# llm-d/llm-d-workload-variant-autoscaler

Hardware: AMD Instinct MI355X
Metric: desired-replica accuracy + SLO-attainment %, Llama-3-8B synthetic QPS ramp (higher is better)
Workload: dtype bf16; 1 GPU; model=meta-llama/Llama-3.1-8B, global_batch=256, seq_len=150, parallelism=dp1, device=AMD Radeon Graphics

## Files before the change

### wva_amd/ops/csrc/attention.hip

```cpp
#include "common.h"
#include "launch.h"

#include <type_traits>

#define HEAD_DIM 128
#define MAX_G 8
#define TILE 64
#define NUM_WAVES 4
#define ROW_DW 66
#define S_ROW 65

template <bool KV_FP8>
using kv_elem_t = std::conditional_t<KV_FP8, fp8_t, bf16>;

__device__ __forceinline__ long ws_row_offset(int b, int kvh, int g, int split,
                                              int num_kv_heads, int G,
                                              int num_splits) {
  return ((((long)b * num_kv_heads + kvh) * G + g) * num_splits + split) *
         (2 + HEAD_DIM);
}

__device__ __forceinline__ long pack8_fp8(const float* v, float inv_scale) {
  unsigned int lo = 0, hi = 0;
  lo = __builtin_amdgcn_cvt_pk_fp8_f32(v[0] * inv_scale, v[1] * inv_scale,
                                       lo, false);
  lo = __builtin_amdgcn_cvt_pk_fp8_f32(v[2] * inv_scale, v[3] * inv_scale,
                                       lo, true);
  hi = __builtin_amdgcn_cvt_pk_fp8_f32(v[4] * inv_scale, v[5] * inv_scale,
                                       hi, false);
  hi = __builtin_amdgcn_cvt_pk_fp8_f32(v[6] * inv_scale, v[7] * inv_scale,
                                       hi, true);
  return (long)(((unsigned long)hi << 32) | lo);
}

struct QFrags {
  bf16x8_frag bf[4];
  long fp8[4];
  float scale;
};

template <bool KV_FP8>
__device__ __forceinline__ QFrags load_q_frags(const bf16* __restrict__ q,
                                               int b, int kvh, int G,
                                               int num_q_heads, int lane,
                                               int wave, int g, int k0,
                                               float* qmax_lds) {
  QFrags qf;
  qf.scale = 1.0f;
#pragma unroll
  for (int kk = 0; kk < 4; ++kk) qf.fp8[kk] = 0;
  float qv[4][8];
#pragma unroll
  for (int kk = 0; kk < 4; ++kk)
#pragma unroll
    for (int i = 0; i < 8; ++i) qv[kk][i] = 0.0f;
  if (g < G) {
    const bf16* qrow = q + ((long)b * num_q_heads + kvh * G + g) * HEAD_DIM;
#pragma unroll
    for (int kk = 0; kk < 4; ++kk) {
      const short* src = reinterpret_cast<const short*>(qrow + 32 * kk + k0);
#pragma unroll
      for (int i = 0; i < 8; ++i) {
        qf.bf[kk][i] = src[i];
        const bf16 bv = *reinterpret_cast<const bf16*>(&src[i]);
        qv[kk][i] = bf2f(bv);
      }
    }
  } else {
#pragma unroll
    for (int kk = 0; kk < 4; ++kk)
#pragma unroll
      for (int i = 0; i < 8; ++i) qf.bf[kk][i] = 0;
  }
  if constexpr (KV_FP8) {
    float amax = 0.0f;
#pragma unroll
    for (int kk = 0; kk < 4; ++kk)
#pragma unroll
      for (int i = 0; i < 8; ++i) amax = fmaxf(amax, fabsf(qv[kk][i]));
    amax = wave_reduce_max(amax);
    if (lane == 0) qmax_lds[wave] = amax;
    __syncthreads();
    float m0 = qmax_lds[0];
#pragma unroll
    for (int w2 = 1; w2 < NUM_WAVES; ++w2) m0 = fmaxf(m0, qmax_lds[w2]);
    qf.scale = fmaxf(m0 / 448.0f, 1e-12f);
    const float inv = 1.0f / qf.scale;
#pragma unroll
    for (int kk = 0; kk < 4; ++kk) qf.fp8[kk] = pack8_fp8(qv[kk], inv);
    __syncthreads();
  }
  return qf;
}

struct SoftmaxStep {
  float p;
  float corr;
};

__device__ __forceinline__ SoftmaxStep online_softmax_step(
    const float* __restrict__ s_row, int tn, int lane, float& m, float& s) {
  const bool live = lane < tn;
  const float score = live ? s_row[lane] : -INFINITY;
  const float tile_max = wave_reduce_max(score);
  const float m_new = fmaxf(m, tile_max);
  const float p = live ? __expf(score - m_new) : 0.0f;
  const float tile_sum = wave_reduce_sum(p);
  const float corr = (m == -INFINITY) ? 0.0f : __expf(m - m_new);
  s = s * corr + tile_sum;
  m = m_new;
  return {p, corr};
}


struct TilePages {
  int id[4];

  __device__ __forceinline__ int pick(int group) const {
    return group == 0 ? id[0] : group == 1 ? id[1] : group == 2 ? id[2] : id[3];
  }
};

__device__ __forceinline__ TilePages load_tile_pages(
    const int* __restrict__ table_row, int t0, int ctx, int block_shift,
    int num_blocks) {
  const int last_block = (ctx - 1) >> block_shift;
  TilePages pages;
#pragma unroll
  for (int g = 0; g < 4; ++g) {
    const int entry = min((t0 + 16 * g) >> block_shift, last_block);
    const int id = table_row[entry];
    pages.id[g] = min(max(id, 0), num_blocks - 1);
  }
  return pages;
}

template <typename T>
__device__ __forceinline__ const T* page_row(const T* head0,
                                             const TilePages& pages, int group,
                                             int pos, int block_mask,
                                             long page_stride) {
  return head0 + (long)pages.pick(group) * page_stride +
         (long)(pos & block_mask) * HEAD_DIM;
}

template <bool KV_FP8, bool PAGED>
__global__ __launch_bounds__(256, 2) void gqa_decode_attn_v4_kernel(
    bf16* __restrict__ out,
    float* __restrict__ workspace,
    const bf16* __restrict__ q,
    const void* __restrict__ k_cache,
    const void* __restrict__ v_cache,
    const int* __restrict__ context_lens,
    const int num_q_heads,
    const int num_kv_heads,
    const int max_seq,
    const float scale,
    const int* __restrict__ block_tables,
    const int max_blocks,
    const int block_shift,
    const int num_blocks) {
  const int b = blockIdx.x;
  const int kvh = blockIdx.y;
  const int split = blockIdx.z;
  const int num_splits = gridDim.z;
  const int G = num_q_heads / num_kv_heads;
  const int ctx =
      PAGED ? min(context_lens[b], max_seq) : context_lens[b];

  const int lane = threadIdx.x & (WAVE_SIZE - 1);
  const int wave = threadIdx.x / WAVE_SIZE;
  const int frag_col = lane % 16;
  const int frag_k0 = 8 * (lane / 16);

  __shared__ float s_smem[MAX_G][S_ROW];
  __shared__ unsigned int v_smem[TILE * ROW_DW];
  __shared__ float p_smem[MAX_G][TILE];
  float* qmax_lds = nullptr;
  if constexpr (KV_FP8) {
    __shared__ float qmax_smem[NUM_WAVES];
    qmax_lds = qmax_smem;
  }

  const QFrags qf = load_q_frags<KV_FP8>(q, b, kvh, G, num_q_heads, lane,
                                         wave, frag_col, frag_k0, qmax_lds);

  const int heads_mine = (G > wave) ? (G - wave + NUM_WAVES - 1) / NUM_WAVES : 0;
  float m[2], s[2], acc[2][2];
#pragma unroll
  for (int j = 0; j < 2; ++j) {
    m[j] = -INFINITY;
    s[j] = 0.0f;
    acc[j][0] = acc[j][1] = 0.0f;
  }

  const long slab_off =
      PAGED ? (long)kvh << (block_shift + 7)
            : ((long)b * num_kv_heads + kvh) * max_seq * HEAD_DIM;
  const long page_stride = (long)num_kv_heads << (block_shift + 7);
  const int block_mask = (1 << block_shift) - 1;
  const int* table_row = block_tables + (long)b * max_blocks;
  const auto* k_slab =
      reinterpret_cast<const kv_elem_t<KV_FP8>*>(k_cache) + slab_off;
  const auto* v_slab =
      reinterpret_cast<const kv_elem_t<KV_FP8>*>(v_cache) + slab_off;

  for (int t0 = split * TILE; t0 < ctx; t0 += num_splits * TILE) {
    const int tn = min(TILE, ctx - t0);
    TilePages pages;
    if constexpr (PAGED)
      pages = load_tile_pages(table_row, t0, ctx, block_shift, num_blocks);

    if constexpr (KV_FP8) {
      const int tile_g8 = tn * (HEAD_DIM / 8);
      const fp8_t* v_src = v_slab + (long)t0 * HEAD_DIM;
      for (int idx = wave * WAVE_SIZE + lane; idx < tile_g8;
           idx += NUM_WAVES * WAVE_SIZE) {
        const int row = idx >> 4;
        const int d8 = (idx & 15) * 8;
        const fp8_t* v_row;
        if constexpr (PAGED)
          v_row = page_row(v_slab, pages,
                           __builtin_amdgcn_readfirstlane(row >> 4), t0 + row,
                           block_mask, page_stride);
        else
          v_row = v_src + (long)row * HEAD_DIM;
        const unsigned short* src =
            reinterpret_cast<const unsigned short*>(v_row + d8);
        unsigned int* dst = &v_smem[row * ROW_DW + d8 / 2];
#pragma unroll
        for (int j = 0; j < 4; ++j) {
          const float2_vt f = unpk2_fp8(src[j]);
          const bf16x2 packed{f2bf(f[0]), f2bf(f[1])};
          dst[j] = *reinterpret_cast<const unsigned int*>(&packed);
        }
      }
    } else {
      typedef __attribute__((ext_vector_type(2))) unsigned int uint2_t;
      const int tile_u2 = tn * (HEAD_DIM / 4);
      const unsigned int* v_src =
          reinterpret_cast<const unsigned int*>(v_slab + (long)t0 * HEAD_DIM);
      for (int idx = wave * WAVE_SIZE + lane; idx < tile_u2;
           idx += NUM_WAVES * WAVE_SIZE) {
        const int row = idx >> 5;
        const int d2 = (idx & 31) * 2;
        const unsigned int* src;
        if constexpr (PAGED)
          src = reinterpret_cast<const unsigned int*>(page_row(
                    v_slab, pages, __builtin_amdgcn_readfirstlane(row >> 4),
                    t0 + row, block_mask, page_stride)) + d2;
        else
          src = &v_src[idx * 2];
        const uint2_t val = *reinterpret_cast<const uint2_t*>(src);
        *reinterpret_cast<uint2_t*>(&v_smem[row * ROW_DW + d2]) = val;
      }
    }

    {
      const int prow = 16 * wave + (lane % 16);
      const int pos = t0 + prow;
      const int pos_lim = PAGED ? ctx : max_seq;
      const int pos_c = pos < pos_lim ? pos : pos_lim - 1;
      const kv_elem_t<KV_FP8>* k_row;
      if constexpr (PAGED)
        k_row = page_row(k_slab, pages, __builtin_amdgcn_readfirstlane(wave),
                         pos_c, block_mask, page_stride);
      else
        k_row = k_slab + (long)pos_c * HEAD_DIM;
      const int k0 = frag_k0;
      f32x4_frag sf = {0.f, 0.f, 0.f, 0.f};
      if constexpr (KV_FP8) {
        const long* ksrc = reinterpret_cast<const long*>(k_row);
        const int l0 = k0 / 8;
#pragma unroll
        for (int kk = 0; kk < 4; ++kk) {
          const long a8 = ksrc[kk * 4 + l0];
          sf = __builtin_amdgcn_mfma_f32_16x16x32_fp8_fp8(
              a8, qf.fp8[kk], sf, 0, 0, 0);
        }
      } else {
#pragma unroll
        for (int kk = 0; kk < 4; ++kk) {
          bf16x8_frag a_frag;
          const short* src =
              reinterpret_cast<const short*>(k_row) + 32 * kk + k0;
#pragma unroll
          for (int i = 0; i < 8; ++i) a_frag[i] = src[i];
          sf = __builtin_amdgcn_mfma_f32_16x16x32_bf16(a_frag, qf.bf[kk],
                                                       sf, 0, 0, 0);
        }
      }
      const float s_eff = KV_FP8 ? scale * qf.scale : scale;
      const int g = lane & 15;
      if (g < G) {
#pragma unroll
        for (int i = 0; i < 4; ++i) {
          const int t = 16 * wave + (lane >> 4) * 4 + i;
          s_smem[g][t] = (t < tn) ? sf[i] * s_eff : -INFINITY;
        }
      }
    }
    __syncthreads();

    for (int j = 0; j < heads_mine; ++j) {
      const int g = wave + j * NUM_WAVES;
      const SoftmaxStep st = online_softmax_step(s_smem[g], tn, lane, m[j], s[j]);
      acc[j][0] *= st.corr;
      acc[j][1] *= st.corr;
      p_smem[g][lane] = st.p;
    }

    for (int j = 0; j < heads_mine; ++j) {
      const int g = wave + j * NUM_WAVES;
      const float* pg = p_smem[g];
      float a0 = acc[j][0], a1 = acc[j][1];
      for (int t = 0; t < tn; ++t) {
        const unsigned int vw = v_smem[t * ROW_DW + lane];
        const bf16x2 vv = *reinterpret_cast<const bf16x2*>(&vw);
        const float p = pg[t];
        a0 = fmaf(p, bf2f(vv.x), a0);
        a1 = fmaf(p, bf2f(vv.y), a1);
      }
      acc[j][0] = a0;
      acc[j][1] = a1;
    }
    __syncthreads();
  }

  if (num_splits == 1) {
    for (int j = 0; j < heads_mine; ++j) {
      const int g = wave + j * NUM_WAVES;
      const float inv = s[j] > 0.0f ? 1.0f / s[j] : 0.0f;
      bf16x2* orow = reinterpret_cast<bf16x2*>(
          out + ((long)b * num_q_heads + kvh * G + g) * HEAD_DIM);
      orow[lane] = bf16x2{f2bf(acc[j][0] * inv), f2bf(acc[j][1] * inv)};
    }
  } else {
    for (int j = 0; j < heads_mine; ++j) {
      const int g = wave + j * NUM_WAVES;
      float* wsp = workspace +
          ws_row_offset(b, kvh, g, split, num_kv_heads, G, num_splits);
      if (lane == 0) {
        wsp[0] = m[j];
        wsp[1] = s[j];
      }
      wsp[2 + 2 * lane] = acc[j][0];
      wsp[2 + 2 * lane + 1] = acc[j][1];
    }
  }
}

template <bool KV_FP8, bool PAGED>
__global__ __launch_bounds__(256, 2) void gqa_decode_attn_v5_kernel(
    bf16* __restrict__ out,
    float* __restrict__ workspace,
    const bf16* __restrict__ q,
    const void* __restrict__ k_cache,
    const void* __restrict__ v_cache,
    const int* __restrict__ context_lens,
    const int num_q_heads,
    const int num_kv_heads,
    const int max_seq,
    const float scale,
    const int* __restrict__ block_tables,
    const int max_blocks,
    const int block_shift,
    const int num_blocks) {
  const int b = blockIdx.x;
  const int kvh = blockIdx.y;
  const int split = blockIdx.z;
  const int num_splits = gridDim.z;
  const int G = num_q_heads / num_kv_heads;
  const int ctx =
      PAGED ? min(context_lens[b], max_seq) : context_lens[b];

  const int lane = threadIdx.x & (WAVE_SIZE - 1);
  const int wave = threadIdx.x / WAVE_SIZE;
  const int frag_col = lane % 16;
  const int frag_k0 = 8 * (lane / 16);

  __shared__ float s_smem[MAX_G][S_ROW];
  __shared__ unsigned int v_smem[TILE * ROW_DW];
  __shared__ float p_smem[MAX_G][TILE];
  __shared__ float corr_smem[MAX_G];
  __shared__ float sum_smem[MAX_G];
  __shared__ float m_smem[MAX_G];
  float* qmax_lds = nullptr;
  if constexpr (KV_FP8) {
    __shared__ float qmax_smem[NUM_WAVES];
    qmax_lds = qmax_smem;
  }

  const QFrags qf = load_q_frags<KV_FP8>(q, b, kvh, G, num_q_heads, lane,
                                         wave, frag_col, frag_k0, qmax_lds);

  const int heads_mine = (G > wave) ? (G - wave + NUM_WAVES - 1) / NUM_WAVES : 0;
  float m[2], s[2];
#pragma unroll
  for (int j = 0; j < 2; ++j) {
    m[j] = -INFINITY;
    s[j] = 0.0f;
  }
  f32x4_frag acc_pv[2] = {f32x4_frag{0.f, 0.f, 0.f, 0.f},
                          f32x4_frag{0.f, 0.f, 0.f, 0.f}};

  const long slab_off =
      PAGED ? (long)kvh << (block_shift + 7)
            : ((long)b * num_kv_heads + kvh) * max_seq * HEAD_DIM;
  const long page_stride = (long)num_kv_heads << (block_shift + 7);
  const int block_mask = (1 << block_shift) - 1;
  const int* table_row = block_tables + (long)b * max_blocks;
  const auto* k_slab =
      reinterpret_cast<const kv_elem_t<KV_FP8>*>(k_cache) + slab_off;
  const auto* v_slab =
      reinterpret_cast<const kv_elem_t<KV_FP8>*>(v_cache) + slab_off;

  for (int t0 = split * TILE; t0 < ctx; t0 += num_splits * TILE) {
    const int tn = min(TILE, ctx - t0);
    TilePages pages;
    if constexpr (PAGED)
      pages = load_tile_pages(table_row, t0, ctx, block_shift, num_blocks);

    if constexpr (KV_FP8) {
      const int tile_g8 = tn * (HEAD_DIM / 8);
      const fp8_t* v_src = v_slab + (long)t0 * HEAD_DIM;
      for (int idx = wave * WAVE_SIZE + lane; idx < tile_g8;
           idx += NUM_WAVES * WAVE_SIZE) {
        const int row = idx >> 4;
        const int d8 = (idx & 15) * 8;
        const fp8_t* v_row;
        if constexpr (PAGED)
          v_row = page_row(v_slab, pages,
                           __builtin_amdgcn_readfirstlane(row >> 4), t0 + row,
                           block_mask, page_stride);
        else
          v_row = v_src + (long)row * HEAD_DIM;
        const unsigned short* src =
            reinterpret_cast<const unsigned short*>(v_row + d8);
        unsigned int* dst = &v_smem[row * ROW_DW + d8 / 2];
#pragma unroll
        for (int j = 0; j < 4; ++j) {
          const float2_vt f = unpk2_fp8(src[j]);
          const bf16x2 packed{f2bf(f[0]), f2bf(f[1])};
          dst[j] = *reinterpret_cast<const unsigned int*>(&packed);
        }
      }
    } else {
      typedef __attribute__((ext_vector_type(2))) unsigned int uint2_t;
      const int tile_u2 = tn * (HEAD_DIM / 4);
      const unsigned int* v_src =
          reinterpret_cast<const unsigned int*>(v_slab + (long)t0 * HEAD_DIM);
      for (int idx = wave * WAVE_SIZE + lane; idx < tile_u2;
           idx += NUM_WAVES * WAVE_SIZE) {
        const int row = idx >> 5;
        const int d2 = (idx & 31) * 2;
        const unsigned int* src;
        if constexpr (PAGED)
          src = reinterpret_cast<const unsigned int*>(page_row(
                    v_slab, pages, __builtin_amdgcn_readfirstlane(row >> 4),
                    t0 + row, block_mask, page_stride)) + d2;
        else
          src = &v_src[idx * 2];
        const uint2_t val = *reinterpret_cast<const uint2_t*>(src);
        *reinterpret_cast<uint2_t*>(&v_smem[row * ROW_DW + d2]) = val;
      }
    }

    {
      const int prow = 16 * wave + (lane % 16);
      const int pos = t0 + prow;
      const int pos_lim = PAGED ? ctx : max_seq;
      const int pos_c = pos < pos_lim ? pos : pos_lim - 1;
      const kv_elem_t<KV_FP8>* k_row;
      if constexpr (PAGED)
        k_row = page_row(k_slab, pages, __builtin_amdgcn_readfirstlane(wave),
                         pos_c, block_mask, page_stride);
      else
        k_row = k_slab + (long)pos_c * HEAD_DIM;
      const int k0 = frag_k0;
      f32x4_frag sf = {0.f, 0.f, 0.f, 0.f};
      if constexpr (KV_FP8) {
        const long* ksrc = reinterpret_cast<const long*>(k_row);
        const int l0 = k0 / 8;
#pragma unroll
        for (int kk = 0; kk < 4; ++kk) {
          const long a8 = ksrc[kk * 4 + l0];
          sf = __builtin_amdgcn_mfma_f32_16x16x32_fp8_fp8(
              a8, qf.fp8[kk], sf, 0, 0, 0);
        }
      } else {
#pragma unroll
        for (int kk = 0; kk < 4; ++kk) {
          bf16x8_frag a_frag;
          const short* src =
              reinterpret_cast<const short*>(k_row) + 32 * kk + k0;
#pragma unroll
          for (int i = 0; i < 8; ++i) a_frag[i] = src[i];
          sf = __builtin_amdgcn_mfma_f32_16x16x32_bf16(a_frag, qf.bf[kk],
                                                       sf, 0, 0, 0);
        }
      }
      const float s_eff = KV_FP8 ? scale * qf.scale : scale;
      const int g = lane & 15;
      if (g < G) {
#pragma unroll
        for (int i = 0; i < 4; ++i) {
          const int t = 16 * wave + (lane >> 4) * 4 + i;
          s_smem[g][t] = (t < tn) ? sf[i] * s_eff : -INFINITY;
        }
      }
    }
    __syncthreads();

    for (int j = 0; j < heads_mine; ++j) {
      const int g = wave + j * NUM_WAVES;
      const SoftmaxStep st = online_softmax_step(s_smem[g], tn, lane, m[j], s[j]);
      p_smem[g][lane] = st.p;
      if (lane == 0) corr_smem[g] = st.corr;
    }
    __syncthreads();

    {
      bf16x8_frag p_frag[2];
#pragma unroll
      for (int kk = 0; kk < 2; ++kk) {
        const int g = lane % 16;
        const int pos0 = 32 * kk + 8 * (lane / 16);
        if (g < G) {
#pragma unroll
          for (int i = 0; i < 8; ++i)
            p_frag[kk][i] = f2bf_bits(p_smem[g][pos0 + i]);
        } else {
#pragma unroll
          for (int i = 0; i < 8; ++i) p_frag[kk][i] = 0;
        }
      }
      const unsigned short* v_u16 =
          reinterpret_cast<const unsigned short*>(v_smem);
#pragma unroll
      for (int nsub = 0; nsub < 2; ++nsub) {
        const int dim = 16 * (wave + 4 * nsub) + (lane % 16);
        f32x4_frag d = acc_pv[nsub];
#pragma unroll
        for (int i = 0; i < 4; ++i) {
          const int h = (lane >> 4) * 4 + i;
          d[i] *= (h < G) ? corr_smem[h] : 0.0f;
        }
#pragma unroll
        for (int kk = 0; kk < 2; ++kk) {
          bf16x8_frag v_frag;
          const int pos0 = 32 * kk + 8 * (lane / 16);
#pragma unroll
          for (int i = 0; i < 8; ++i) {
            const int t = pos0 + i;
            v_frag[i] = (t < tn)
                ? (short)v_u16[(t * ROW_DW + (dim >> 1)) * 2 + (dim & 1)]
                : (short)0;
          }
          d = __builtin_amdgcn_mfma_f32_16x16x32_bf16(p_frag[kk], v_frag, d,
                                                      0, 0, 0);
        }
        acc_pv[nsub] = d;
      }
    }
    __syncthreads();
  }

  for (int j = 0; j < heads_mine; ++j) {
    const int g = wave + j * NUM_WAVES;
    if (lane == 0) {
      sum_smem[g] = s[j];
      m_smem[g] = m[j];
    }
  }
  __syncthreads();

  if (num_splits == 1) {
#pragma unroll
    for (int nsub = 0; nsub < 2; ++nsub) {
      const int dim = 16 * (wave + 4 * nsub) + (lane & 15);
#pragma unroll
      for (int i = 0; i < 4; ++i) {
        const int h = (lane >> 4) * 4 + i;
        if (h >= G) continue;
        const float sv = sum_smem[h];
        const float inv = sv > 0.0f ? 1.0f / sv : 0.0f;
        out[((long)b * num_q_heads + kvh * G + h) * HEAD_DIM + dim] =
            f2bf(acc_pv[nsub][i] * inv);
      }
    }
  } else {
#pragma unroll
    for (int nsub = 0; nsub < 2; ++nsub) {
      const int dim = 16 * (wave + 4 * nsub) + (lane & 15);
#pragma unroll
      for (int i = 0; i < 4; ++i) {
        const int h = (lane >> 4) * 4 + i;
        if (h >= G) continue;
        float* wsp = workspace +
            ws_row_offset(b, kvh, h, split, num_kv_heads, G, num_splits);
        if (wave == 0 && nsub == 0 && (lane & 15) == 0) {
          wsp[0] = m_smem[h];
          wsp[1] = sum_smem[h];
        }
        wsp[2 + dim] = acc_pv[nsub][i];
      }
    }
  }
}

#define MERGE_WAVES 8
__global__ __launch_bounds__(64 * MERGE_WAVES) void gqa_decode_attn_merge_kernel(
    bf16* __restrict__ out,
    const float* __restrict__ workspace,
    const int num_q_heads,
    const int num_kv_heads,
    const int num_splits) {
  const int b = blockIdx.x;
  const int h = blockIdx.y;
  const int G = num_q_heads / num_kv_heads;
  const int kvh = h / G;
  const int g = h % G;
  const int lane = threadIdx.x & 63;
  const int wave = threadIdx.x >> 6;

  __shared__ float sm_m[MERGE_WAVES];
  __shared__ float sm_s[MERGE_WAVES];
  __shared__ float sm_o[MERGE_WAVES][HEAD_DIM];

  const float* base = workspace +
      ws_row_offset(b, kvh, g, 0, num_kv_heads, G, num_splits);
  float M = -INFINITY;
  for (int sp = wave; sp < num_splits; sp += MERGE_WAVES) {
    M = fmaxf(M, base[sp * (2 + HEAD_DIM)]);
  }
  float S = 0.0f, o0 = 0.0f, o1 = 0.0f;
  for (int sp = wave; sp < num_splits; sp += MERGE_WAVES) {
    const float* wsp = base + sp * (2 + HEAD_DIM);
    const float mw = wsp[0];
    if (mw == -INFINITY) continue;
    const float f = __expf(mw - M);
    S += wsp[1] * f;
    o0 = fmaf(wsp[2 + 2 * lane], f, o0);
    o1 = fmaf(wsp[2 + 2 * lane + 1], f, o1);
  }
  if (lane == 0) {
    sm_m[wave] = M;
    sm_s[wave] = S;
  }
  sm_o[wave][2 * lane] = o0;
  sm_o[wave][2 * lane + 1] = o1;
  __syncthreads();

  if (wave != 0) return;
  float Mg = -INFINITY;
  for (int w = 0; w < MERGE_WAVES; ++w) Mg = fmaxf(Mg, sm_m[w]);
  float Sg = 0.0f;
  float g0 = 0.0f, g1 = 0.0f;
  for (int w = 0; w < MERGE_WAVES; ++w) {
    if (sm_m[w] == -INFINITY) continue;
    const float f = __expf(sm_m[w] - Mg);
    Sg += sm_s[w] * f;
    g0 = fmaf(sm_o[w][2 * lane], f, g0);
    g1 = fmaf(sm_o[w][2 * lane + 1], f, g1);
  }
  const float inv = Sg > 0.0f ? 1.0f / Sg : 0.0f;
  bf16x2* orow = reinterpret_cast<bf16x2*>(
      out + ((long)b * num_q_heads + h) * HEAD_DIM);
  orow[lane] = bf16x2{f2bf(g0 * inv), f2bf(g1 * inv)};
}

extern "C" int gqa_decode_attn_num_splits(int batch, int num_kv_heads,
                                          int max_ctx_hint) {
  const int base = batch * num_kv_heads;
  if (base >= 1792) return 1;
  int splits = 1792 / base;
  static int min_tiles = [] {
    const char* e = getenv("WVA_ATTN_MIN_TILES");
    int v = e ? atoi(e) : 8;
    return v > 0 ? v : 8;
  }();
  int cap = 16;
  if (max_ctx_hint > 0) {
    const int by_work = max_ctx_hint / (min_tiles * TILE);
    if (by_work > cap) cap = by_work;
  }
  if (splits > cap) splits = cap;
  const int max_useful = max_ctx_hint > 0 ? (max_ctx_hint + 2 * TILE - 1) / (2 * TILE) : splits;
  if (splits > max_useful && max_useful >= 1) splits = max_useful;
  return splits < 1 ? 1 : splits;
}

template <bool PAGED>
static auto decode_attn_kernel(int variant, int kv_fp8) {
  return variant == 5 ? (kv_fp8 ? gqa_decode_attn_v5_kernel<true, PAGED>
                                : gqa_decode_attn_v5_kernel<false, PAGED>)
                      : (kv_fp8 ? gqa_decode_attn_v4_kernel<true, PAGED>
                                : gqa_decode_attn_v4_kernel<false, PAGED>);
}

extern "C" void launch_gqa_decode_attn(
    void* out, void* workspace, const void* q, const void* k_cache,
    const void* v_cache, const int* context_lens, const PagedKV* paged,
    int batch, int num_q_heads, int num_kv_heads, int max_seq, int num_splits,
    float scale, int variant, int kv_fp8, hipStream_t stream) {
  const auto kernel = !paged ? decode_attn_kernel<false>(variant, kv_fp8)
                             : decode_attn_kernel<true>(variant, kv_fp8);
  const PagedKV p = paged ? *paged : PagedKV{nullptr, 0, 0, 0};
  if (paged) max_seq = p.max_blocks << p.block_shift;
  hipLaunchKernelGGL(kernel, dim3(batch, num_kv_heads, num_splits), dim3(256),
                     0, stream, (bf16*)out, (float*)workspace, (const bf16*)q,
                     k_cache, v_cache, context_lens, num_q_heads, num_kv_heads,
                     max_seq, scale, p.block_tables, p.max_blocks,
                     p.block_shift, p.num_blocks);
  if (num_splits > 1) {
    hipLaunchKernelGGL(gqa_decode_attn_merge_kernel,
                       dim3(batch, num_q_heads), dim3(64 * MERGE_WAVES), 0,
                       stream, (bf16*)out, (const float*)workspace,
                       num_q_heads, num_kv_heads, num_splits);
  }
}
```

### wva_amd/ops/csrc/rmsnorm.hip

```cpp

#include "common.h"
#include "launch.h"

typedef __attribute__((ext_vector_type(4))) float floatx4;

template <bool HAS_RESIDUAL>
__global__ void rmsnorm_kernel(
    bf16* __restrict__ out,
    bf16* __restrict__ residual_out,
    const bf16* __restrict__ input,
    const bf16* __restrict__ residual,
    const bf16* __restrict__ weight,
    const float eps,
    const int hidden) {
  const int row = blockIdx.x;
  const bf16* in_row = input + (long)row * hidden;
  const bf16* res_row = HAS_RESIDUAL ? residual + (long)row * hidden : nullptr;
  bf16* out_row = out + (long)row * hidden;
  bf16* res_out_row =
      HAS_RESIDUAL ? residual_out + (long)row * hidden : nullptr;

  __shared__ float lds_red[16];

  float ss = 0.0f;
  const int vec_n = hidden / 8;
  const bf16x2* in2 = reinterpret_cast<const bf16x2*>(in_row);
  const bf16x2* res2 =
      HAS_RESIDUAL ? reinterpret_cast<const bf16x2*>(res_row) : nullptr;
  bf16x2* res_out2 =
      HAS_RESIDUAL ? reinterpret_cast<bf16x2*>(res_out_row) : nullptr;

  for (int i = threadIdx.x; i < vec_n; i += blockDim.x) {
#pragma unroll
    for (int j = 0; j < 4; ++j) {
      bf16x2 v = in2[i * 4 + j];
      float lo = bf2f(v.x), hi = bf2f(v.y);
      if (HAS_RESIDUAL) {
        bf16x2 r = res2[i * 4 + j];
        lo += bf2f(r.x);
        hi += bf2f(r.y);
        res_out2[i * 4 + j] = bf16x2{f2bf(lo), f2bf(hi)};
      }
      ss = fmaf(lo, lo, ss);
      ss = fmaf(hi, hi, ss);
    }
  }
  ss = block_reduce_sum(ss, lds_red);
  const float inv_rms = rsqrtf(ss / (float)hidden + eps);
  __syncthreads();

  const bf16x2* x2 = HAS_RESIDUAL ? reinterpret_cast<const bf16x2*>(res_out_row)
                                  : in2;
  const bf16x2* w2 = reinterpret_cast<const bf16x2*>(weight);
  bf16x2* o2 = reinterpret_cast<bf16x2*>(out_row);
  for (int i = threadIdx.x; i < vec_n; i += blockDim.x) {
#pragma unroll
    for (int j = 0; j < 4; ++j) {
      bf16x2 v = x2[i * 4 + j];
      bf16x2 w = w2[i * 4 + j];
      o2[i * 4 + j] = bf16x2{
          f2bf(bf2f(v.x) * inv_rms * bf2f(w.x)),
          f2bf(bf2f(v.y) * inv_rms * bf2f(w.y))};
    }
  }
}

extern "C" void launch_rmsnorm(
    void* out, void* residual_out, const void* input, const void* residual,
    const void* weight, float eps, int rows, int hidden, hipStream_t stream) {
  dim3 grid(rows);
  dim3 block(256);
  if (residual != nullptr) {
    hipLaunchKernelGGL(rmsnorm_kernel<true>, grid, block, 0, stream,
                       (bf16*)out, (bf16*)residual_out, (const bf16*)input,
                       (const bf16*)residual, (const bf16*)weight, eps, hidden);
  } else {
    hipLaunchKernelGGL(rmsnorm_kernel<false>, grid, block, 0, stream,
                       (bf16*)out, nullptr, (const bf16*)input, nullptr,
                       (const bf16*)weight, eps, hidden);
  }
}
```

### wva_amd/ops/csrc/rope.hip

```cpp

#include "common.h"
#include "launch.h"

__device__ __forceinline__ void rotate_pair(
    const bf16* src, bf16* dst, int d, int half, int head_dim, float pos,
    float theta) {
  const float inv_freq = __powf(theta, -2.0f * (float)d / (float)head_dim);
  const float angle = pos * inv_freq;
  float c, s;
  __sincosf(angle, &s, &c);
  const float x1 = bf2f(src[d]);
  const float x2 = bf2f(src[d + half]);
  dst[d] = f2bf(x1 * c - x2 * s);
  dst[d + half] = f2bf(x2 * c + x1 * s);
}

struct RopeCosSin {
  float c;
  float s;
};

__device__ __forceinline__ RopeCosSin rope_cos_sin(int d, int head_dim,
                                                   int pos,
                                                   double log2_theta) {
  const double inv_freq =
      exp2(-2.0 * (double)d / (double)head_dim * log2_theta);
  double turns = (double)pos * inv_freq * 0.15915494309189535;
  turns -= floor(turns);
  const float t = (float)turns;
  return {__builtin_amdgcn_cosf(t), __builtin_amdgcn_sinf(t)};
}

struct RopeCosSinCache {
  int d = -1;
  RopeCosSin cs = {1.0f, 0.0f};

  __device__ __forceinline__ RopeCosSin get(int d_new, int head_dim, int pos,
                                            double log2_theta) {
    if (d_new != d) {
      cs = rope_cos_sin(d_new, head_dim, pos, log2_theta);
      d = d_new;
    }
    return cs;
  }
};

__device__ __forceinline__ void rotate_pair_cs(
    const bf16* src, bf16* dst, int d, int half, RopeCosSin cs) {
  const float x1 = bf2f(src[d]);
  const float x2 = bf2f(src[d + half]);
  dst[d] = f2bf(x1 * cs.c - x2 * cs.s);
  dst[d + half] = f2bf(x2 * cs.c + x1 * cs.s);
}

__device__ __forceinline__ long paged_row_offset(
    const int* __restrict__ block_tables, int b, int pos, int max_blocks,
    int block_shift, int num_blocks, int num_kv_heads, int head_dim) {
  const int entry = pos >> block_shift;
  if (pos < 0 || entry >= max_blocks) return -1;
  const int id = block_tables[(long)b * max_blocks + entry];
  if (id < 0 || id >= num_blocks) return -1;
  const long row = (((long)id * num_kv_heads) << block_shift) +
                   (pos & ((1 << block_shift) - 1));
  return row * head_dim;
}

__global__ void rope_kernel(
    bf16* __restrict__ q,
    bf16* __restrict__ k,
    const int* __restrict__ positions,
    const int num_q_heads,
    const int num_k_heads,
    const int head_dim,
    const float theta) {
  const int token = blockIdx.x;
  const float pos = (float)positions[token];
  const int half = head_dim / 2;
  const int total = (num_q_heads + num_k_heads) * half;

  for (int idx = threadIdx.x; idx < total; idx += blockDim.x) {
    const int head = idx / half;
    const int d = idx % half;
    const bool is_q = head < num_q_heads;
    bf16* base = is_q
        ? q + (long)token * num_q_heads * head_dim + (long)head * head_dim
        : k + (long)token * num_k_heads * head_dim +
              (long)(head - num_q_heads) * head_dim;
    rotate_pair(base, base, d, half, head_dim, pos, theta);
  }
}

template <bool PAGED>
__global__ void rope_append_kv_kernel(
    const bf16* __restrict__ qkv,
    bf16* __restrict__ q_out,
    bf16* __restrict__ k_cache,
    bf16* __restrict__ v_cache,
    const int* __restrict__ positions,
    const int num_q_heads,
    const int num_kv_heads,
    const int head_dim,
    const int max_seq,
    const float theta,
    const int* __restrict__ block_tables,
    const int max_blocks,
    const int block_shift,
    const int num_blocks) {
  const int b = blockIdx.x;
  const int pos_i = positions[b];
  const float pos = (float)pos_i;
  const int half = head_dim / 2;
  const long qkv_row = (long)b * (num_q_heads + 2 * num_kv_heads) * head_dim;
  const long row0 =
      PAGED ? paged_row_offset(block_tables, b, pos_i, max_blocks, block_shift,
                               num_blocks, num_kv_heads, head_dim)
            : ((long)b * num_kv_heads * max_seq + pos_i) * head_dim;
  const long head_stride =
      PAGED ? (long)head_dim << block_shift : (long)max_seq * head_dim;
  const bool has_row = !PAGED || row0 >= 0;

  const int rot_total = (num_q_heads + num_kv_heads) * half;
  for (int idx = threadIdx.x; idx < rot_total; idx += blockDim.x) {
    const int head = idx / half;
    const int d = idx % half;
    if (head < num_q_heads) {
      const bf16* src = qkv + qkv_row + (long)head * head_dim;
      bf16* dst = q_out + ((long)b * num_q_heads + head) * head_dim;
      rotate_pair(src, dst, d, half, head_dim, pos, theta);
    } else {
      const int kh = head - num_q_heads;
      const bf16* src = qkv + qkv_row + ((long)num_q_heads + kh) * head_dim;
      bf16* dst = k_cache + row0 + kh * head_stride;
      if (has_row) rotate_pair(src, dst, d, half, head_dim, pos, theta);
    }
  }
  const int v_total = num_kv_heads * half;
  const bf16x2* vsrc = reinterpret_cast<const bf16x2*>(
      qkv + qkv_row + (long)(num_q_heads + num_kv_heads) * head_dim);
  for (int idx = threadIdx.x; idx < v_total; idx += blockDim.x) {
    const int kh = idx / half;
    const int d2 = idx % half;
    bf16x2* dst =
        reinterpret_cast<bf16x2*>(v_cache + row0 + kh * head_stride);
    if (has_row) dst[d2] = vsrc[(long)kh * half + d2];
  }
}

template <bool PAGED>
__global__ void rope_append_kv_fp8_kernel(
    const bf16* __restrict__ qkv,
    bf16* __restrict__ q_out,
    fp8_t* __restrict__ k_cache,
    fp8_t* __restrict__ v_cache,
    const int* __restrict__ positions,
    const int num_q_heads,
    const int num_kv_heads,
    const int head_dim,
    const int max_seq,
    const double log2_theta,
    const int* __restrict__ block_tables,
    const int max_blocks,
    const int block_shift,
    const int num_blocks) {
  const int b = blockIdx.x;
  const int pos_i = positions[b];
  const int half = head_dim / 2;
  const long qkv_row = (long)b * (num_q_heads + 2 * num_kv_heads) * head_dim;
  const long row0 =
      PAGED ? paged_row_offset(block_tables, b, pos_i, max_blocks, block_shift,
                               num_blocks, num_kv_heads, head_dim)
            : ((long)b * num_kv_heads * max_seq + pos_i) * head_dim;
  const long head_stride =
      PAGED ? (long)head_dim << block_shift : (long)max_seq * head_dim;
  const bool has_row = !PAGED || row0 >= 0;

  const int rot_total = (num_q_heads + num_kv_heads) * half;
  RopeCosSinCache cache;
  for (int idx = threadIdx.x; idx < rot_total; idx += blockDim.x) {
    const int head = idx / half;
    const int d = idx % half;
    const RopeCosSin cs = cache.get(d, head_dim, pos_i, log2_theta);
    if (head < num_q_heads) {
      const bf16* src = qkv + qkv_row + (long)head * head_dim;
      bf16* dst = q_out + ((long)b * num_q_heads + head) * head_dim;
      rotate_pair_cs(src, dst, d, half, cs);
    } else {
      const int kh = head - num_q_heads;
      const bf16* src = qkv + qkv_row + ((long)num_q_heads + kh) * head_dim;
      const float x1 = bf2f(src[d]);
      const float x2 = bf2f(src[d + half]);
      fp8_t* dst = k_cache + row0 + kh * head_stride;
      if (has_row) {
        dst[d] = f2fp8(x1 * cs.c - x2 * cs.s);
        dst[d + half] = f2fp8(x2 * cs.c + x1 * cs.s);
      }
    }
  }
  const int v_total = num_kv_heads * half;
  const bf16x2* vsrc = reinterpret_cast<const bf16x2*>(
      qkv + qkv_row + (long)(num_q_heads + num_kv_heads) * head_dim);
  for (int idx = threadIdx.x; idx < v_total; idx += blockDim.x) {
    const int kh = idx / half;
    const int d2 = idx % half;
    const bf16x2 v2 = vsrc[(long)kh * half + d2];
    unsigned short* dst =
        reinterpret_cast<unsigned short*>(v_cache + row0 + kh * head_stride);
    if (has_row) dst[d2] = pk2_fp8(bf2f(v2.x), bf2f(v2.y));
  }
}

extern "C" void launch_rope(
    void* q, void* k, const int* positions, int tokens, int num_q_heads,
    int num_k_heads, int head_dim, float theta, hipStream_t stream) {
  dim3 grid(tokens);
  dim3 block(256);
  hipLaunchKernelGGL(rope_kernel, grid, block, 0, stream, (bf16*)q, (bf16*)k,
                     positions, num_q_heads, num_k_heads, head_dim, theta);
}

template <bool PAGED>
static void launch_append_kernel(
    const void* qkv, void* q_out, void* k_cache, void* v_cache,
    const int* positions, const PagedKV& p, int batch, int num_q_heads,
    int num_kv_heads, int head_dim, int max_seq, float theta, int kv_fp8,
    hipStream_t stream) {
  dim3 grid(batch);
  dim3 block(256);
  if (kv_fp8) {
    hipLaunchKernelGGL(rope_append_kv_fp8_kernel<PAGED>, grid, block, 0,
                       stream, (const bf16*)qkv, (bf16*)q_out, (fp8_t*)k_cache,
                       (fp8_t*)v_cache, positions, num_q_heads, num_kv_heads,
                       head_dim, max_seq, log2((double)theta), p.block_tables,
                       p.max_blocks, p.block_shift, p.num_blocks);
  } else {
    hipLaunchKernelGGL(rope_append_kv_kernel<PAGED>, grid, block, 0, stream,
                       (const bf16*)qkv, (bf16*)q_out, (bf16*)k_cache,
                       (bf16*)v_cache, positions, num_q_heads, num_kv_heads,
                       head_dim, max_seq, theta, p.block_tables, p.max_blocks,
                       p.block_shift, p.num_blocks);
  }
}

extern "C" void launch_rope_append_kv(
    const void* qkv, void* q_out, void* k_cache, void* v_cache,
    const int* positions, const PagedKV* paged, int batch, int num_q_heads,
    int num_kv_heads, int head_dim, int max_seq, float theta, int kv_fp8,
    hipStream_t stream) {
  if (!paged) {
    launch_append_kernel<false>(qkv, q_out, k_cache, v_cache, positions,
                                PagedKV{nullptr, 0, 0, 0}, batch, num_q_heads,
                                num_kv_heads, head_dim, max_seq, theta, kv_fp8,
                                stream);
  } else {
    launch_append_kernel<true>(qkv, q_out, k_cache, v_cache, positions,
                               *paged, batch, num_q_heads, num_kv_heads,
                               head_dim, 0, theta, kv_fp8, stream);
  }
}
```

### wva_amd/ops/csrc/silu_mul.hip

```cpp

#include "common.h"
#include "launch.h"

__global__ void silu_mul_kernel(
    bf16* __restrict__ out,
    const bf16* __restrict__ gate,
    const bf16* __restrict__ up,
    const long n2) {
  const bf16x2* g2 = reinterpret_cast<const bf16x2*>(gate);
  const bf16x2* u2 = reinterpret_cast<const bf16x2*>(up);
  bf16x2* o2 = reinterpret_cast<bf16x2*>(out);
  const long stride = (long)gridDim.x * blockDim.x;
  for (long i = (long)blockIdx.x * blockDim.x + threadIdx.x; i < n2;
       i += stride) {
    bf16x2 g = g2[i];
    bf16x2 u = u2[i];
    const float glo = bf2f(g.x), ghi = bf2f(g.y);
    const float slo = glo / (1.0f + __expf(-glo));
    const float shi = ghi / (1.0f + __expf(-ghi));
    o2[i] = bf16x2{f2bf(slo * bf2f(u.x)), f2bf(shi * bf2f(u.y))};
  }
}

__global__ void silu_mul_fused_kernel(
    bf16* __restrict__ out,
    const bf16* __restrict__ gate_up,
    const long rows,
    const long inter2) {
  const long n2 = rows * inter2;
  const long stride = (long)gridDim.x * blockDim.x;
  bf16x2* o2 = reinterpret_cast<bf16x2*>(out);
  const bf16x2* gu2 = reinterpret_cast<const bf16x2*>(gate_up);
  for (long i = (long)blockIdx.x * blockDim.x + threadIdx.x; i < n2;
       i += stride) {
    const long row = i / inter2;
    const long col = i % inter2;
    const bf16x2 g = gu2[row * 2 * inter2 + col];
    const bf16x2 u = gu2[row * 2 * inter2 + inter2 + col];
    const float glo = bf2f(g.x), ghi = bf2f(g.y);
    const float slo = glo / (1.0f + __expf(-glo));
    const float shi = ghi / (1.0f + __expf(-ghi));
    o2[i] = bf16x2{f2bf(slo * bf2f(u.x)), f2bf(shi * bf2f(u.y))};
  }
}

static int silu_grid(long n2) {
  long want = (n2 + 255) / 256;
  return (int)(want > 8192 ? 8192 : (want < 1 ? 1 : want));
}

extern "C" void launch_silu_mul(
    void* out, const void* gate, const void* up, long n, hipStream_t stream) {
  const long n2 = n / 2;
  hipLaunchKernelGGL(silu_mul_kernel, dim3(silu_grid(n2)), dim3(256), 0,
                     stream, (bf16*)out, (const bf16*)gate, (const bf16*)up,
                     n2);
}

extern "C" void launch_silu_mul_fused(
    void* out, const void* gate_up, long rows, long inter, hipStream_t stream) {
  const long inter2 = inter / 2;
  hipLaunchKernelGGL(silu_mul_fused_kernel, dim3(silu_grid(rows * inter2)),
                     dim3(256), 0, stream, (bf16*)out, (const bf16*)gate_up,
                     rows, inter2);
}
```

Measured before the change: 91.98 %.

## Vectorize rmsnorm, rope, silu_mul kernels and add small-split attention merge

Adds 16-byte vectorized variants of rmsnorm (holding the row in registers so it is read once), rope-append-KV (a shared-memory cos/sin table with 128-bit loads and stores), and silu_mul (plain and fused). It also caches cos/sin per dimension in the scalar rope paths and adds a lighter attention merge kernel that packs four rows per block when the split count is small. Each path is chosen only when pointers are 16-byte aligned and the shapes fit. The aim is fewer memory transactions and less launch and compute overhead in these small, memory-bound kernels. The changes also add more code paths and rely on alignment checks, and the new merge kernel replaces the original merge path whenever the split count is small.

```diff
diff --git a/wva_amd/ops/csrc/attention.hip b/wva_amd/ops/csrc/attention.hip
--- a/wva_amd/ops/csrc/attention.hip
+++ b/wva_amd/ops/csrc/attention.hip
@@ -670,6 +670,36 @@
   orow[lane] = bf16x2{f2bf(g0 * inv), f2bf(g1 * inv)};
 }
 
+#define MERGE_ROWS 4
+__global__ __launch_bounds__(64 * MERGE_ROWS) void gqa_decode_attn_merge_small_kernel(
+    bf16* __restrict__ out,
+    const float* __restrict__ workspace,
+    const int rows,
+    const int num_splits) {
+  const int lane = threadIdx.x & 63;
+  const int row = blockIdx.x * MERGE_ROWS + (threadIdx.x >> 6);
+  if (row >= rows) return;
+  const float* base = workspace + (long)row * num_splits * (2 + HEAD_DIM);
+  float Mg = -INFINITY;
+  for (int sp = 0; sp < num_splits; ++sp) {
+    Mg = fmaxf(Mg, fmaxf(-INFINITY, base[sp * (2 + HEAD_DIM)]));
+  }
+  float Sg = 0.0f;
+  float g0 = 0.0f, g1 = 0.0f;
+  for (int sp = 0; sp < num_splits; ++sp) {
+    const float* wsp = base + sp * (2 + HEAD_DIM);
+    const float m = fmaxf(-INFINITY, wsp[0]);
+    if (m == -INFINITY) continue;
+    const float f = __expf(m - Mg);
+    Sg += wsp[1] * f;
+    g0 = fmaf(wsp[2 + 2 * lane], f, g0);
+    g1 = fmaf(wsp[2 + 2 * lane + 1], f, g1);
+  }
+  const float inv = Sg > 0.0f ? 1.0f / Sg : 0.0f;
+  bf16x2* orow = reinterpret_cast<bf16x2*>(out + (long)row * HEAD_DIM);
+  orow[lane] = bf16x2{f2bf(g0 * inv), f2bf(g1 * inv)};
+}
+
 extern "C" int gqa_decode_attn_num_splits(int batch, int num_kv_heads,
                                           int max_ctx_hint) {
   const int base = batch * num_kv_heads;
@@ -713,7 +743,13 @@
                      k_cache, v_cache, context_lens, num_q_heads, num_kv_heads,
                      max_seq, scale, p.block_tables, p.max_blocks,
                      p.block_shift, p.num_blocks);
-  if (num_splits > 1) {
+  if (num_splits > 1 && num_splits <= MERGE_WAVES) {
+    const int rows = batch * num_q_heads;
+    hipLaunchKernelGGL(gqa_decode_attn_merge_small_kernel,
+                       dim3((rows + MERGE_ROWS - 1) / MERGE_ROWS),
+                       dim3(64 * MERGE_ROWS), 0, stream, (bf16*)out,
+                       (const float*)workspace, rows, num_splits);
+  } else if (num_splits > 1) {
     hipLaunchKernelGGL(gqa_decode_attn_merge_kernel,
                        dim3(batch, num_q_heads), dim3(64 * MERGE_WAVES), 0,
                        stream, (bf16*)out, (const float*)workspace,
diff --git a/wva_amd/ops/csrc/rmsnorm.hip b/wva_amd/ops/csrc/rmsnorm.hip
--- a/wva_amd/ops/csrc/rmsnorm.hip
+++ b/wva_amd/ops/csrc/rmsnorm.hip
@@ -1,3 +1,5 @@
+
+#include <cstdint>
 
 #include "common.h"
 #include "launch.h"
@@ -65,11 +67,114 @@
   }
 }
 
+typedef __attribute__((ext_vector_type(4))) unsigned int u32x4;
+#define RMS_REG_VECS 4
+#define RMS_REG_MAX (RMS_REG_VECS * 256 * 8)
+
+__device__ __forceinline__ float rms_lo(unsigned int w) {
+  return __uint_as_float(w << 16);
+}
+__device__ __forceinline__ float rms_hi(unsigned int w) {
+  return __uint_as_float(w & 0xffff0000u);
+}
+__device__ __forceinline__ unsigned int rms_pack(float lo, float hi) {
+  return (unsigned int)(unsigned short)f2bf_bits(lo) |
+         ((unsigned int)(unsigned short)f2bf_bits(hi) << 16);
+}
+
+template <bool HAS_RESIDUAL>
+__global__ __launch_bounds__(256) void rmsnorm_reg_kernel(
+    bf16* __restrict__ out,
+    bf16* __restrict__ residual_out,
+    const bf16* __restrict__ input,
+    const bf16* __restrict__ residual,
+    const bf16* __restrict__ weight,
+    const float eps,
+    const int hidden) {
+  const int row = blockIdx.x;
+  const int vec_n = hidden / 8;
+  const u32x4* in8 =
+      reinterpret_cast<const u32x4*>(input + (long)row * hidden);
+  const u32x4* res8 = HAS_RESIDUAL ? reinterpret_cast<const u32x4*>(
+                                         residual + (long)row * hidden)
+                                   : nullptr;
+  u32x4* res_out8 = HAS_RESIDUAL ? reinterpret_cast<u32x4*>(
+                                       residual_out + (long)row * hidden)
+                                 : nullptr;
+  const u32x4* w8 = reinterpret_cast<const u32x4*>(weight);
+  u32x4* o8 = reinterpret_cast<u32x4*>(out + (long)row * hidden);
+
+  __shared__ float lds_red[16];
+
+  u32x4 x[RMS_REG_VECS], r[RMS_REG_VECS], w[RMS_REG_VECS];
+#pragma unroll
+  for (int k = 0; k < RMS_REG_VECS; ++k) {
+    const int i = threadIdx.x + 256 * k;
+    if (i < vec_n) {
+      x[k] = in8[i];
+      if (HAS_RESIDUAL) r[k] = res8[i];
+      w[k] = w8[i];
+    }
+  }
+
+  float ss = 0.0f;
+#pragma unroll
+  for (int k = 0; k < RMS_REG_VECS; ++k) {
+    const int i = threadIdx.x + 256 * k;
+    if (i < vec_n) {
+#pragma unroll
+      for (int j = 0; j < 4; ++j) {
+        float lo = rms_lo(x[k][j]), hi = rms_hi(x[k][j]);
+        if (HAS_RESIDUAL) {
+          lo += rms_lo(r[k][j]);
+          hi += rms_hi(r[k][j]);
+          x[k][j] = rms_pack(lo, hi);
+        }
+        ss = fmaf(lo, lo, ss);
+        ss = fmaf(hi, hi, ss);
+      }
+      if (HAS_RESIDUAL) res_out8[i] = x[k];
+    }
+  }
+  ss = block_reduce_sum(ss, lds_red);
+  const float inv_rms = rsqrtf(ss / (float)hidden + eps);
+
+#pragma unroll
+  for (int k = 0; k < RMS_REG_VECS; ++k) {
+    const int i = threadIdx.x + 256 * k;
+    if (i < vec_n) {
+      u32x4 o;
+#pragma unroll
+      for (int j = 0; j < 4; ++j) {
+        o[j] = rms_pack(rms_lo(x[k][j]) * inv_rms * rms_lo(w[k][j]),
+                        rms_hi(x[k][j]) * inv_rms * rms_hi(w[k][j]));
+      }
+      o8[i] = o;
+    }
+  }
+}
+
 extern "C" void launch_rmsnorm(
     void* out, void* residual_out, const void* input, const void* residual,
     const void* weight, float eps, int rows, int hidden, hipStream_t stream) {
   dim3 grid(rows);
   dim3 block(256);
+  const bool aligned =
+      (((uintptr_t)out | (uintptr_t)residual_out | (uintptr_t)input |
+        (uintptr_t)residual | (uintptr_t)weight) & 15) == 0;
+  if (hidden <= RMS_REG_MAX && aligned) {
+    if (residual != nullptr) {
+      hipLaunchKernelGGL(rmsnorm_reg_kernel<true>, grid, block, 0, stream,
+                         (bf16*)out, (bf16*)residual_out, (const bf16*)input,
+                         (const bf16*)residual, (const bf16*)weight, eps,
+                         hidden);
+    } else {
+      hipLaunchKernelGGL(rmsnorm_reg_kernel<false>, grid, block, 0, stream,
+                         (bf16*)out, nullptr, (const bf16*)input, nullptr,
+                         (const bf16*)weight, eps, hidden);
+    }
+    return;
+  }
   if (residual != nullptr) {
     hipLaunchKernelGGL(rmsnorm_kernel<true>, grid, block, 0, stream,
                        (bf16*)out, (bf16*)residual_out, (const bf16*)input,
diff --git a/wva_amd/ops/csrc/rope.hip b/wva_amd/ops/csrc/rope.hip
--- a/wva_amd/ops/csrc/rope.hip
+++ b/wva_amd/ops/csrc/rope.hip
@@ -1,24 +1,52 @@
+
+#include <cstdint>
 
 #include "common.h"
 #include "launch.h"
 
-__device__ __forceinline__ void rotate_pair(
-    const bf16* src, bf16* dst, int d, int half, int head_dim, float pos,
-    float theta) {
+struct RopeCosSin {
+  float c;
+  float s;
+};
+
+__device__ __forceinline__ RopeCosSin rope_cos_sin_f32(int d, int head_dim,
+                                                       float pos,
+                                                       float theta) {
   const float inv_freq = __powf(theta, -2.0f * (float)d / (float)head_dim);
   const float angle = pos * inv_freq;
   float c, s;
   __sincosf(angle, &s, &c);
+  return {c, s};
+}
+
+__device__ __forceinline__ float rope_lo(float x1, float x2, RopeCosSin cs) {
+  return fmaf(cs.c, x1, -__fmul_rn(cs.s, x2));
+}
+__device__ __forceinline__ float rope_hi(float x1, float x2, RopeCosSin cs) {
+  return fmaf(cs.s, x1, __fmul_rn(cs.c, x2));
+}
+
+struct RopeCosSinCacheF32 {
+  int d = -1;
+  RopeCosSin cs = {1.0f, 0.0f};
+
+  __device__ __forceinline__ RopeCosSin get(int d_new, int head_dim,
+                                            float pos, float theta) {
+    if (d_new != d) {
+      cs = rope_cos_sin_f32(d_new, head_dim, pos, theta);
+      d = d_new;
+    }
+    return cs;
+  }
+};
+
+__device__ __forceinline__ void rotate_pair(
+    const bf16* src, bf16* dst, int d, int half, RopeCosSin cs) {
   const float x1 = bf2f(src[d]);
   const float x2 = bf2f(src[d + half]);
-  dst[d] = f2bf(x1 * c - x2 * s);
-  dst[d + half] = f2bf(x2 * c + x1 * s);
-}
-
-struct RopeCosSin {
-  float c;
-  float s;
-};
+  dst[d] = f2bf(rope_lo(x1, x2, cs));
+  dst[d + half] = f2bf(rope_hi(x1, x2, cs));
+}
 
 __device__ __forceinline__ RopeCosSin rope_cos_sin(int d, int head_dim,
                                                    int pos,
@@ -78,6 +106,7 @@
   const int half = head_dim / 2;
   const int total = (num_q_heads + num_k_heads) * half;
 
+  RopeCosSinCacheF32 cache;
   for (int idx = threadIdx.x; idx < total; idx += blockDim.x) {
     const int head = idx / half;
     const int d = idx % half;
@@ -86,7 +115,7 @@
         ? q + (long)token * num_q_heads * head_dim + (long)head * head_dim
         : k + (long)token * num_k_heads * head_dim +
               (long)(head - num_q_heads) * head_dim;
-    rotate_pair(base, base, d, half, head_dim, pos, theta);
+    rotate_pair(base, base, d, half, cache.get(d, head_dim, pos, theta));
   }
 }
 
@@ -120,18 +149,20 @@
   const bool has_row = !PAGED || row0 >= 0;
 
   const int rot_total = (num_q_heads + num_kv_heads) * half;
+  RopeCosSinCacheF32 cache;
   for (int idx = threadIdx.x; idx < rot_total; idx += blockDim.x) {
     const int head = idx / half;
     const int d = idx % half;
+    const RopeCosSin cs = cache.get(d, head_dim, pos, theta);
     if (head < num_q_heads) {
       const bf16* src = qkv + qkv_row + (long)head * head_dim;
       bf16* dst = q_out + ((long)b * num_q_heads + head) * head_dim;
-      rotate_pair(src, dst, d, half, head_dim, pos, theta);
+      rotate_pair(src, dst, d, half, cs);
     } else {
       const int kh = head - num_q_heads;
       const bf16* src = qkv + qkv_row + ((long)num_q_heads + kh) * head_dim;
       bf16* dst = k_cache + row0 + kh * head_stride;
-      if (has_row) rotate_pair(src, dst, d, half, head_dim, pos, theta);
+      if (has_row) rotate_pair(src, dst, d, half, cs);
     }
   }
   const int v_total = num_kv_heads * half;
@@ -143,6 +174,106 @@
     bf16x2* dst =
         reinterpret_cast<bf16x2*>(v_cache + row0 + kh * head_stride);
     if (has_row) dst[d2] = vsrc[(long)kh * half + d2];
+  }
+}
+
+typedef __attribute__((ext_vector_type(4))) unsigned int u32x4;
+#define ROPE_VEC_LANES 64
+
+__device__ __forceinline__ float bf_lo(unsigned int w) {
+  return __uint_as_float(w << 16);
+}
+__device__ __forceinline__ float bf_hi(unsigned int w) {
+  return __uint_as_float(w & 0xffff0000u);
+}
+__device__ __forceinline__ unsigned int pack_bf2(float lo, float hi) {
+  return (unsigned int)(unsigned short)f2bf_bits(lo) |
+         ((unsigned int)(unsigned short)f2bf_bits(hi) << 16);
+}
+
+template <bool PAGED>
+__global__ __launch_bounds__(ROPE_VEC_LANES) void rope_append_kv_vec_kernel(
+    const bf16* __restrict__ qkv,
+    bf16* __restrict__ q_out,
+    bf16* __restrict__ k_cache,
+    bf16* __restrict__ v_cache,
+    const int* __restrict__ positions,
+    const int num_q_heads,
+    const int num_kv_heads,
+    const int head_dim,
+    const int max_seq,
+    const float theta,
+    const int* __restrict__ block_tables,
+    const int max_blocks,
+    const int block_shift,
+    const int num_blocks) {
+  __shared__ float tab_c[ROPE_VEC_LANES];
+  __shared__ float tab_s[ROPE_VEC_LANES];
+
+  const int b = blockIdx.x;
+  const int lane = threadIdx.x;
+  const int item = blockIdx.y * ROPE_VEC_LANES + lane;
+  const int rot_items = (num_q_heads + num_kv_heads) * 8;
+  const int total = rot_items + num_kv_heads * 16;
+  const bool is_rot = item < rot_items;
+  const bool is_v = !is_rot && item < total;
+  const bf16* row =
+      qkv + (long)b * (num_q_heads + 2 * num_kv_heads) * 128;
+
+  int head = 0, j = 0;
+  u32x4 a = {0u, 0u, 0u, 0u}, h = {0u, 0u, 0u, 0u};
+  if (is_rot) {
+    head = item >> 3;
+    j = item & 7;
+    const bf16* src = row + (long)head * 128 + j * 8;
+    a = *reinterpret_cast<const u32x4*>(src);
+    h = *reinterpret_cast<const u32x4*>(src + 64);
+  } else if (is_v) {
+    head = (item - rot_items) >> 4;
+    j = (item - rot_items) & 15;
+    a = *reinterpret_cast<const u32x4*>(
+        row + (long)(num_q_heads + num_kv_heads + head) * 128 + j * 8);
+  }
+
+  const int pos_i = positions[b];
+  const long row0 =
+      PAGED ? paged_row_offset(block_tables, b, pos_i, max_blocks, block_shift,
+                               num_blocks, num_kv_heads, head_dim)
+            : ((long)b * num_kv_heads * max_seq + pos_i) * head_dim;
+  const long head_stride =
+      PAGED ? (long)head_dim << block_shift : (long)max_seq * head_dim;
+  const bool has_row = !PAGED || row0 >= 0;
+
+  {
+    const RopeCosSin cs = rope_cos_sin_f32(lane, head_dim, (float)pos_i, theta);
+    tab_c[lane] = cs.c;
+    tab_s[lane] = cs.s;
+  }
+  __syncthreads();
+
+  if (is_rot) {
+    bf16* dst;
+    if (head < num_q_heads) {
+      dst = q_out + ((long)b * num_q_heads + head) * 128;
+    } else {
+      if (!has_row) return;
+      dst = k_cache + row0 + (head - num_q_heads) * head_stride;
+    }
+    u32x4 lo, hi;
+#pragma unroll
+    for (int w = 0; w < 4; ++w) {
+      const RopeCosSin c0 = {tab_c[j * 8 + 2 * w], tab_s[j * 8 + 2 * w]};
+      const RopeCosSin c1 = {tab_c[j * 8 + 2 * w + 1],
+                             tab_s[j * 8 + 2 * w + 1]};
+      const float x1a = bf_lo(a[w]), x1b = bf_hi(a[w]);
+      const float x2a = bf_lo(h[w]), x2b = bf_hi(h[w]);
+      lo[w] = pack_bf2(rope_lo(x1a, x2a, c0), rope_lo(x1b, x2b, c1));
+      hi[w] = pack_bf2(rope_hi(x1a, x2a, c0), rope_hi(x1b, x2b, c1));
+    }
+    *reinterpret_cast<u32x4*>(dst + j * 8) = lo;
+    *reinterpret_cast<u32x4*>(dst + 64 + j * 8) = hi;
+  } else if (is_v && has_row) {
+    *reinterpret_cast<u32x4*>(v_cache + row0 + head * head_stride + j * 8) = a;
   }
 }
 
@@ -218,6 +349,12 @@
                      positions, num_q_heads, num_k_heads, head_dim, theta);
 }
 
+static bool aligned16(const void* a, const void* b, const void* c,
+                      const void* d) {
+  return (((uintptr_t)a | (uintptr_t)b | (uintptr_t)c | (uintptr_t)d) & 15) ==
+         0;
+}
+
 template <bool PAGED>
 static void launch_append_kernel(
     const void* qkv, void* q_out, void* k_cache, void* v_cache,
@@ -232,6 +369,15 @@
                        (fp8_t*)v_cache, positions, num_q_heads, num_kv_heads,
                        head_dim, max_seq, log2((double)theta), p.block_tables,
                        p.max_blocks, p.block_shift, p.num_blocks);
+  } else if (head_dim == 128 && aligned16(qkv, q_out, k_cache, v_cache)) {
+    const int items = (num_q_heads + num_kv_heads) * 8 + num_kv_heads * 16;
+    const int parts = (items + ROPE_VEC_LANES - 1) / ROPE_VEC_LANES;
+    hipLaunchKernelGGL(rope_append_kv_vec_kernel<PAGED>, dim3(batch, parts),
+                       dim3(ROPE_VEC_LANES), 0, stream, (const bf16*)qkv,
+                       (bf16*)q_out, (bf16*)k_cache, (bf16*)v_cache, positions,
+                       num_q_heads, num_kv_heads, head_dim, max_seq, theta,
+                       p.block_tables, p.max_blocks, p.block_shift,
+                       p.num_blocks);
   } else {
     hipLaunchKernelGGL(rope_append_kv_kernel<PAGED>, grid, block, 0, stream,
                        (const bf16*)qkv, (bf16*)q_out, (bf16*)k_cache,
diff --git a/wva_amd/ops/csrc/silu_mul.hip b/wva_amd/ops/csrc/silu_mul.hip
--- a/wva_amd/ops/csrc/silu_mul.hip
+++ b/wva_amd/ops/csrc/silu_mul.hip
@@ -1,3 +1,5 @@
+
+#include <cstdint>
 
 #include "common.h"
 #include "launch.h"
@@ -44,13 +46,74 @@
   }
 }
 
+typedef __attribute__((ext_vector_type(4))) unsigned int u32x4;
+
+__device__ __forceinline__ unsigned int silu_mul_pair(unsigned int g,
+                                                      unsigned int u) {
+  const float glo = __uint_as_float(g << 16);
+  const float ghi = __uint_as_float(g & 0xffff0000u);
+  const float slo = glo / (1.0f + __expf(-glo));
+  const float shi = ghi / (1.0f + __expf(-ghi));
+  const float olo = slo * __uint_as_float(u << 16);
+  const float ohi = shi * __uint_as_float(u & 0xffff0000u);
+  return (unsigned int)(unsigned short)f2bf_bits(olo) |
+         ((unsigned int)(unsigned short)f2bf_bits(ohi) << 16);
+}
+
+__device__ __forceinline__ u32x4 silu_mul_vec(u32x4 g, u32x4 u) {
+  u32x4 o;
+#pragma unroll
+  for (int w = 0; w < 4; ++w) o[w] = silu_mul_pair(g[w], u[w]);
+  return o;
+}
+
+__global__ void silu_mul_vec_kernel(
+    bf16* __restrict__ out,
+    const bf16* __restrict__ gate,
+    const bf16* __restrict__ up,
+    const long n8) {
+  const u32x4* g8 = reinterpret_cast<const u32x4*>(gate);
+  const u32x4* u8 = reinterpret_cast<const u32x4*>(up);
+  u32x4* o8 = reinterpret_cast<u32x4*>(out);
+  const long stride = (long)gridDim.x * blockDim.x;
+  for (long i = (long)blockIdx.x * blockDim.x + threadIdx.x; i < n8;
+       i += stride) {
+    o8[i] = silu_mul_vec(g8[i], u8[i]);
+  }
+}
+
+__global__ void silu_mul_fused_vec_kernel(
+    bf16* __restrict__ out,
+    const bf16* __restrict__ gate_up,
+    const long rows,
+    const int inter8) {
+  const int col = blockIdx.x * blockDim.x + threadIdx.x;
+  if (col >= inter8) return;
+  const u32x4* gu8 = reinterpret_cast<const u32x4*>(gate_up);
+  u32x4* o8 = reinterpret_cast<u32x4*>(out);
+  for (long row = blockIdx.y; row < rows; row += gridDim.y) {
+    const u32x4* in = gu8 + row * 2 * inter8;
+    o8[row * inter8 + col] = silu_mul_vec(in[col], in[inter8 + col]);
+  }
+}
+
 static int silu_grid(long n2) {
   long want = (n2 + 255) / 256;
   return (int)(want > 8192 ? 8192 : (want < 1 ? 1 : want));
 }
 
+static bool silu_aligned16(const void* a, const void* b, const void* c) {
+  return (((uintptr_t)a | (uintptr_t)b | (uintptr_t)c) & 15) == 0;
+}
+
 extern "C" void launch_silu_mul(
     void* out, const void* gate, const void* up, long n, hipStream_t stream) {
+  if (n % 8 == 0 && silu_aligned16(out, gate, up)) {
+    hipLaunchKernelGGL(silu_mul_vec_kernel, dim3(silu_grid(n / 8)), dim3(256),
+                       0, stream, (bf16*)out, (const bf16*)gate,
+                       (const bf16*)up, n / 8);
+    return;
+  }
   const long n2 = n / 2;
   hipLaunchKernelGGL(silu_mul_kernel, dim3(silu_grid(n2)), dim3(256), 0,
                      stream, (bf16*)out, (const bf16*)gate, (const bf16*)up,
@@ -59,6 +122,16 @@
 
 extern "C" void launch_silu_mul_fused(
     void* out, const void* gate_up, long rows, long inter, hipStream_t stream) {
+  if (rows > 0 && inter > 0 && inter % 8 == 0 && inter / 8 < (1L << 30) &&
+      silu_aligned16(out, gate_up, nullptr)) {
+    const int inter8 = (int)(inter / 8);
+    const long gy = rows > 65535 ? 65535 : rows;
+    hipLaunchKernelGGL(silu_mul_fused_vec_kernel,
+                       dim3((inter8 + 255) / 256, (int)gy), dim3(256), 0,
+                       stream, (bf16*)out,
+                       (const bf16*)gate_up, rows, inter8);
+    return;
+  }
   const long inter2 = inter / 2;
   hipLaunchKernelGGL(silu_mul_fused_kernel, dim3(silu_grid(rows * inter2)),
                      dim3(256), 0, stream, (bf16*)out, (const bf16*)gate_up,
```

After: 91.98 %. Within noise of the previous version (+0.0%).
